# sarulab-speech/visual-onoma-to-wave

Hardware: AMD Instinct MI355X
Metric: end-to-end audio samples/sec (22.05 kHz) + mel-frames/sec, batch 32, 1->8 GPU (higher is better)
Workload: dtype bf16 (encoder+variance adaptor fp32); 1 GPU; C2+C3 end-to-end: vTTS (B, T_src=12, teacher-forced T_mel=512, predicted energy) -> HiFi-GAN V1 generator -> B x 131072 samples; model=vTTS (35.3M) + HiFi-GAN V1 (13.9M), global_batch=32, per_gpu_batch=32, seq_len=512, src_len=12, parallelism=replicas x1 (no data-path collective), pipeline=acoustic(batch i+1) on its own stream || vocoder(batch i)

## Files before the change

### include/vonoma.h

```cpp
#ifndef VONOMA_H_
#define VONOMA_H_

#include <stdint.h>
#ifndef __cplusplus
#include <stdbool.h>
#endif

#ifdef __cplusplus
extern "C" {
#endif

#define VO_OK 0
#define VO_ERR_INVALID (-1)
#define VO_NOT_HANDLED (-2)

enum vo_dtype { VO_F32 = 0, VO_BF16 = 1, VO_F32X3 = 2  };
enum vo_act { VO_ACT_NONE = 0, VO_ACT_RELU = 1, VO_ACT_LRELU = 2, VO_ACT_TANH = 3 };

const char* vo_last_error(void);
#define VO_ABI_VERSION 3
int vo_version(void);
int vo_num_symbols(void);
const char* vo_symbol_name(int i);
int vo_tune(const char* key, int value);
// ... 4 lines not shown
  int64_t x_bstride;
  int ldx;
  const void* w;
  const float* bias;
  void* y;
  int y_dtype;
  int64_t y_bstride;
  int ldy;
  const void* res1;
  const void* res2;
  int B, T_in, T_out;
  int Ci, Co;
  int K, dil, pad;
  int pre_act;  float pre_slope;
  int post_act; float post_slope;
  float out_scale;
  int compute_dtype;
  int transposed, up_stride, up_pad, up_cout, up_tout;
  int variant;
  int stride;
  int groups;
  void* workspace;
  int64_t workspace_bytes;
  const void* ymask;
  float ymask_slope;
  const int32_t* lens;
  int lens_scale;
} vo_conv1d_desc;
int vo_conv1d(const vo_conv1d_desc* d, void* stream);
int64_t vo_conv1d_workspace_size(const vo_conv1d_desc* d);
#define VO_CONV1D_LAUNCH_FIELDS 13
int vo_conv1d_last_launch(int32_t* rec, int n);
int vo_conv1d_plan(const vo_conv1d_desc* d, int32_t* rec, int n);

enum vo_pack_mode { VO_PACK_CONV = 0, VO_PACK_CONVT = 1, VO_PACK_DGRAD = 2 };
int vo_pack_weight(const float* src, const float* g, const float* row_scale, int mode, int Co,
                   int Ci, int K, int stride, void* dst, int dst_dtype, void* stream);

int vo_layernorm(const void* x, int x_dtype, const void* res, int res_dtype, const float* gamma,
                 const float* beta, const int32_t* lens, int B, int T, int D, float eps, void* y,
                 int y_dtype, void* stream);

int vo_layernorm_dual(const void* x, int x_dtype, const void* res, int res_dtype, const float* gamma,
                      const float* beta, const int32_t* lens, int B, int T, int D, float eps, void* y,
                      void* y16, void* stream);

int64_t vo_layernorm_bwd_workspace_size(int B, int T, int D);
int vo_layernorm_bwd(const void* x, const void* res, int x_dtype, const void* gy, int gy_dtype,
                     const float* gamma, const int32_t* lens, int B, int T, int D, float eps, void* gh,
                     float* dgamma, float* dbeta, void* workspace, void* stream);

int vo_layernorm_bwd_ex(const void* x, int x_dtype, const void* res, int res_dtype, const void* gy, int gy_dtype,
                        const void* gy2, const float* gamma, const int32_t* lens, int B, int T, int D, float eps,
                        void* gh, float* gh32, float* dgamma, float* dbeta, void* workspace, void* stream);

int vo_layernorm_drop(const void* x, int x_dtype, const void* res, int res_dtype, const float* gamma,
                      const float* beta, const int32_t* lens, int B, int T, int D, float eps, void* y, int y_dtype,
                      void* y16, float p, const int64_t* seed, unsigned salt, void* stream);
int vo_layernorm_bwd_drop(const void* x, int x_dtype, const void* res, int res_dtype, const void* gy, int gy_dtype,
                          const void* gy2, const float* gamma, const int32_t* lens, int B, int T, int D, float eps,
                          float p, const int64_t* seed, unsigned salt, void* gh, void* gres, float* dgamma,
                          float* dbeta, void* workspace, void* stream);

int vo_attention(const void* qkv, int dtype, const int32_t* lens, int B, int L, int H, int dk,
                 float scale, void* out, void* stream);

// ... 237 lines not shown
```

### visual_onoma_to_wave_amd/_lib.py

```python

import ctypes
import os

_HERE = os.path.dirname(os.path.abspath(__file__))
LIB_PATH = os.environ.get("VO_LIB_PATH") or os.path.join(_HERE, "lib", "libvonoma.so")

VO_F32, VO_BF16, VO_F32X3 = 0, 1, 2
ACT_NONE, ACT_RELU, ACT_LRELU, ACT_TANH = 0, 1, 2, 3
PACK_CONV, PACK_CONVT = 0, 1
HEAD_DURATION, HEAD_ENERGY = 0, 1

c_void_p = ctypes.c_void_p
c_int = ctypes.c_int
c_float = ctypes.c_float
c_int64 = ctypes.c_int64


class Conv1dDesc(ctypes.Structure):
    _fields_ = [
        ("x", c_void_p), ("x_dtype", c_int), ("x_bstride", c_int64), ("ldx", c_int),
        ("w", c_void_p), ("bias", c_void_p),
        ("y", c_void_p), ("y_dtype", c_int), ("y_bstride", c_int64), ("ldy", c_int),
        ("res1", c_void_p), ("res2", c_void_p),
        ("B", c_int), ("T_in", c_int), ("T_out", c_int),
# ... 63 lines not shown
    "vo_num_symbols": (c_int, []),
    "vo_symbol_name": (ctypes.c_char_p, [c_int]),
    "vo_tune": (c_int, [ctypes.c_char_p, c_int]),
    "vo_resblock_pair": (c_int, [c_void_p, c_void_p, c_void_p, c_void_p, c_void_p, c_void_p, c_void_p, c_int,
                                 c_int, c_int, c_int, c_int, c_float, c_float, c_void_p]),
    "vo_resblock_pair_frag": (c_int, [c_void_p, c_void_p, c_void_p, c_void_p, c_void_p, c_void_p, c_void_p, c_int,
                                      c_int, c_int, c_int, c_int, c_float, c_float, c_void_p]),
    "vo_pack_frag": (c_int, [c_void_p, c_void_p, c_int, c_int, c_void_p]),
    "vo_resblock_pair_lens": (c_int, [c_void_p, c_void_p, c_void_p, c_void_p, c_void_p, c_void_p, c_void_p, c_int,
                                      c_int, c_int, c_int, c_int, c_float, c_float, c_void_p, c_void_p, c_int]),
    "vo_resblock_pair_frag_lens": (c_int, [c_void_p, c_void_p, c_void_p, c_void_p, c_void_p, c_void_p, c_void_p, c_int,
                                           c_int, c_int, c_int, c_int, c_float, c_float, c_void_p, c_void_p, c_int]),
    "vo_resblock3_lens": (c_int, [c_void_p, c_void_p, c_void_p, c_void_p, c_void_p, c_void_p, c_void_p, c_void_p, c_int,
                                  c_int, c_int, c_float, c_float, c_void_p, c_void_p, c_int]),
    "vo_conv_post_lens": (c_int, [c_void_p, c_int, c_void_p, c_float, c_int, c_int, c_int, c_int, c_float,
                                  c_void_p, c_void_p, c_void_p, c_int]),
    "vo_conv_post_pcm16": (c_int, [c_void_p, c_int, c_void_p, c_float, c_int, c_int, c_int, c_int, c_float, c_float,
                                   c_void_p, c_void_p]),
    "vo_conv_post_pcm16_lens": (c_int, [c_void_p, c_int, c_void_p, c_float, c_int, c_int, c_int, c_int, c_float,
                                        c_float, c_void_p, c_void_p, c_void_p, c_int]),
    "vo_resblock3": (c_int, [c_void_p, c_void_p, c_void_p, c_void_p, c_void_p, c_void_p, c_void_p, c_void_p, c_int,
                             c_int, c_int, c_float, c_float, c_void_p]),
    "vo_resblockk": (c_int, [c_void_p, c_void_p, c_void_p, c_void_p, c_void_p, c_int, c_void_p, c_void_p, c_void_p,
                             c_int, c_int, c_int, c_float, c_float, c_void_p]),
    "vo_resblockk_lens": (c_int, [c_void_p, c_void_p, c_void_p, c_void_p, c_void_p, c_int, c_void_p, c_void_p, c_void_p,
                                  c_int, c_int, c_int, c_float, c_float, c_void_p, c_void_p, c_int]),
    "vo_resblockk_tile_rows": (c_int, [c_int]),
    "vo_resblock_pair_tile_rows": (c_int, [c_int, c_int, c_int, c_int]),
    "vo_resblock3_tile_rows": (c_int, [c_int, c_void_p]),
    "vo_conv1d": (c_int, [ctypes.POINTER(Conv1dDesc), c_void_p]),
    "vo_conv1d_workspace_size": (ctypes.c_int64, [ctypes.POINTER(Conv1dDesc)]),
    "vo_conv1d_last_launch": (c_int, [ctypes.POINTER(ctypes.c_int32), c_int]),
    "vo_conv1d_plan": (c_int, [ctypes.POINTER(Conv1dDesc), ctypes.POINTER(ctypes.c_int32), c_int]),
    "vo_pack_weight": (c_int, [c_void_p, c_void_p, c_void_p, c_int, c_int, c_int, c_int, c_int,
                               c_void_p, c_int, c_void_p]),
    "vo_layernorm": (c_int, [c_void_p, c_int, c_void_p, c_int, c_void_p, c_void_p, c_void_p, c_int,
                             c_int, c_int, c_float, c_void_p, c_int, c_void_p]),
    "vo_layernorm_dual": (c_int, [c_void_p, c_int, c_void_p, c_int, c_void_p, c_void_p, c_void_p, c_int,
                                  c_int, c_int, c_float, c_void_p, c_void_p, c_void_p]),
    "vo_layernorm_bwd_workspace_size": (ctypes.c_int64, [c_int, c_int, c_int]),
    "vo_layernorm_bwd": (c_int, [c_void_p, c_void_p, c_int, c_void_p, c_int, c_void_p, c_void_p, c_int, c_int,
                                 c_int, c_float, c_void_p, c_void_p, c_void_p, c_void_p, c_void_p]),
    "vo_layernorm_bwd_ex": (c_int, [c_void_p, c_int, c_void_p, c_int, c_void_p, c_int, c_void_p, c_void_p,
                                    c_void_p, c_int, c_int, c_int, c_float, c_void_p, c_void_p, c_void_p,
                                    c_void_p, c_void_p, c_void_p]),
    "vo_layernorm_drop": (c_int, [c_void_p, c_int, c_void_p, c_int, c_void_p, c_void_p, c_void_p, c_int, c_int,
                                  c_int, c_float, c_void_p, c_int, c_void_p, c_float, c_void_p, ctypes.c_uint,
                                  c_void_p]),
    "vo_layernorm_bwd_drop": (c_int, [c_void_p, c_int, c_void_p, c_int, c_void_p, c_int, c_void_p, c_void_p,
                                      c_void_p, c_int, c_int, c_int, c_float, c_float, c_void_p, ctypes.c_uint,
                                      c_void_p, c_void_p, c_void_p, c_void_p, c_void_p, c_void_p]),
    "vo_attention": (c_int, [c_void_p, c_int, c_void_p, c_int, c_int, c_int, c_int, c_float,
                             c_void_p, c_void_p]),
    "vo_attention_bwd_workspace_size": (ctypes.c_int64, [c_int, c_int, c_int]),
    "vo_attention_bwd": (c_int, [c_void_p, c_void_p, c_void_p, c_int, c_void_p, c_int, c_int, c_int, c_int, c_float,
                                 c_void_p, c_void_p, c_void_p]),
    "vo_attention_lse": (c_int, [c_void_p, c_int, c_void_p, c_int, c_int, c_int, c_int, c_float, c_void_p, c_void_p,
                                 c_void_p]),
    "vo_attention_bwd_lse": (c_int, [c_void_p, c_void_p, c_void_p, c_int, c_void_p, c_int, c_int, c_int, c_int,
                                     c_float, c_void_p, c_void_p, c_void_p, c_void_p]),
    "vo_length_regulate": (c_int, [c_void_p, c_int, c_void_p, c_int, c_int, c_int, c_int, c_void_p,
                                   c_int, c_void_p, c_void_p, c_void_p]),
    "vo_length_regulate_bwd": (c_int, [c_void_p, c_int, c_void_p, c_int, c_int, c_int, c_int, c_void_p, c_int,
                                       c_void_p]),
    "vo_lr_lengths": (c_int, [c_void_p, c_int, c_int, c_void_p, c_void_p, c_void_p]),
    "vo_variance_head": (c_int, [ctypes.POINTER(HeadDesc), c_void_p]),
# ... 124 lines not shown
```

### visual_onoma_to_wave_amd/csrc/conv1d.hip

```cpp

#include <string.h>

#include <algorithm>
#include <type_traits>

#include "vo_common.h"

namespace vo {

constexpr int KC = 32;
constexpr int HALO_MAX = 64;

struct ConvArgs {
  const void* x; int64_t xbs; int ldx;
  const void* w; const float* bias;
  void* y; int64_t ybs; int ldy;
  const void* res1; const void* res2;
  int T_in, T_out, Ci, Co, K, dil, pad;
  int pre_act; float pre_slope; int post_act; float post_slope; float out_scale;
  int transposed, up_stride, up_pad, up_cout, up_tout;
  int tiles_per_b, co_tiles, B;
  int cig, cog;
  float* partial;
  int kcs;
// ... 88 lines not shown
      const int pos = min(t0 + wave_t0 + 16 * (j0 + jj) + lr, a.T_out - 1);
      const int64_t off = (int64_t)pos * a.ldy + n0;
#pragma unroll
      for (int h = 0; h < NH; ++h) {
        if (r1) rv1[jj][h] = *reinterpret_cast<const uint4*>(R1 + off + 8 * h);
        if (r2) rv2[jj][h] = *reinterpret_cast<const uint4*>(R2 + off + 8 * h);
        if (om) rvm[jj][h] = *reinterpret_cast<const uint4*>(YM + off + 8 * h);
      }
    }
#pragma unroll
    for (int jj = 0; jj < JG; ++jj) {
      const int j = j0 + jj;
      const int pos = t0 + wave_t0 + 16 * j + lr;
      const int64_t off = (int64_t)min(pos, a.T_out - 1) * a.ldy + n0;
#pragma unroll
      for (int h = 0; h < NH; ++h) {
        float q[8], x1[8], x2[8];
        if (r1) {
          const uint32_t w[4] = {rv1[jj][h].x, rv1[jj][h].y, rv1[jj][h].z, rv1[jj][h].w};
#pragma unroll
          for (int u = 0; u < 4; ++u) {
            x1[2 * u] = __uint_as_float(w[u] << 16);
            x1[2 * u + 1] = __uint_as_float(w[u] & 0xffff0000u);
          }
        }
        if (r2) {
          const uint32_t w[4] = {rv2[jj][h].x, rv2[jj][h].y, rv2[jj][h].z, rv2[jj][h].w};
#pragma unroll
          for (int u = 0; u < 4; ++u) {
            x2[2 * u] = __uint_as_float(w[u] << 16);
            x2[2 * u + 1] = __uint_as_float(w[u] & 0xffff0000u);
          }
        }
#pragma unroll
        for (int e = 0; e < 8; ++e) {
          const int i = 2 * h + e / 4, r = e & 3;
          float v = acc[i][j][r] + bias[8 * h + e];
          v = tanh_act ? tanhf(v) : lrelu_max(v, ps);
          if (r1) v += x1[e];
          v *= a.out_scale;
          if (r2) v += x2[e];
          q[e] = v;
        }
        if (om) {
          const uint32_t w[4] = {rvm[jj][h].x, rvm[jj][h].y, rvm[jj][h].z, rvm[jj][h].w};
#pragma unroll
          for (int e = 0; e < 8; ++e) {
            const float m = __uint_as_float((e & 1) ? (w[e >> 1] & 0xffff0000u) : (w[e >> 1] << 16));
            const float r = to_f32(from_f32<bf16_t>(q[e]));
            q[e] = m > 0.f ? r : r * a.ymask_slope;
          }
        }
        if (pos < a.T_out) store8(Y + off + 8 * h, q);
      }
    }
  }
}

template <typename TOUT, int NI, int NJ, int EJ = 2>
__device__ __forceinline__ void conv_epilogue(const ConvArgs& a, f32x4 (&acc)[NI][NJ], int b, int t0, int co_blk,
                                              int wave_co0, int wave_t0, int lane) {
  const int lr = lane & 15;
  const int g = lane >> 4;
  const int n0 = co_blk + wave_co0 + NI * 4 * g;
  if (n0 >= a.Co) return;
  if constexpr (std::is_same<TOUT, bf16_t>::value && NI % 2 == 0) {
    if (!a.transposed && (a.ldy & 7) == 0 && (a.ybs & 7) == 0 && a.Co % (4 * NI) == 0) {
      conv_epilogue_vec<NI, NJ, EJ>(a, acc, b, t0, n0, wave_t0, lr);
      return;
    }
  }
  TOUT* Y = reinterpret_cast<TOUT*>(a.y) + (int64_t)b * a.ybs;
  const TOUT* R1 = a.res1 ? reinterpret_cast<const TOUT*>(a.res1) + (int64_t)b * a.ybs : nullptr;
  const TOUT* R2 = a.res2 ? reinterpret_cast<const TOUT*>(a.res2) + (int64_t)b * a.ybs : nullptr;

  int col = n0, trow_shift = 0;
// ... 668 lines not shown
  bool SEG = false;
  constexpr int bco() const { return 16 * NI * WCO; }
  constexpr int bt() const { return 16 * NJ * WT; }
  constexpr Tile role(int r, int prio = 0) const { Tile t = *this; t.ROLE = r; t.PRIO = prio; return t; }
  constexpr Tile dma(bool rs = false) const { Tile t = *this; t.GL = true; t.RS = rs; return t; }
  constexpr Tile tps(int n) const { Tile t = *this; t.TPS = n; return t; }
  constexpr Tile seg() const { Tile t = *this; t.SEG = true; return t; }
};
constexpr Tile T32x16{1, 1, 2, 1, 4}, T64x16{1, 1, 4, 1, 4}, T128x16{2, 1, 4, 1, 4}, T128x32{2, 2, 4, 1, 4},
    T128x32_n4w2{4, 1, 2, 2, 2}, T32x64{2, 1, 1, 4, 4}, T64x64{2, 2, 2, 2, 2}, T64x64_n4w1{4, 1, 1, 4, 4},
    T128x64{4, 2, 2, 2, 2}, T64x128{2, 4, 2, 2, 2}, T64x128_n4w1{4, 2, 1, 4, 4}, T128x128{4, 4, 2, 2, 2},
    T256x128{4, 4, 4, 2, 2}, T32x256{2, 4, 1, 4, 4}, T64x256{4, 4, 1, 4, 4}, T128x256{4, 4, 2, 4, 2}, T256x256{4, 8, 4, 2, 2};
constexpr Tile T32x64_seg = Tile{1, 2, 2, 2, 1}.seg(), T64x64_seg = Tile{2, 2, 2, 2, 1}.seg(),
               T32x128_seg = Tile{1, 4, 2, 2, 1}.seg(), T64x128_seg = Tile{2, 4, 2, 2, 1}.seg();
constexpr Tile T256x256_mrf0 = T256x256.role(1, 1).dma(), T256x256_mrf0_rs = T256x256.role(1, 1).dma(true),
               T128x128_mrf1 = T128x128.role(2), T64x256_mrf2 = T64x256.role(3), T32x256_mrf3 = T32x256.role(4);
#ifdef VO_ABLATIONS
constexpr Tile A256x256_t1_gl = T256x256.tps(1).dma(), A256x256_t1_rs = T256x256.tps(1).dma(true),
               A128x128_t1_gl = T128x128.tps(1).dma(), A256x256_t1 = T256x256.tps(1), A64x128_t1 = T64x128.tps(1),
               A128x128_mrf0 = T128x128.role(1), A256x256_mrf0_plain = T256x256.role(1),
               A256x256_mrf0_prio = T256x256.role(1, 1), A256x256_mrf0_t3 = T256x256.role(1, 1).tps(3).dma(),
               A256x256_mrf0_t1 = T256x256.role(1, 1).tps(1).dma(), A256x256_mrf0_t1_rs = T256x256.role(1, 1).tps(1).dma(true);
constexpr Tile LIN_64x64{2, 2, 2, 2, 0}, LIN_128x128{4, 4, 2, 2, 0}, LIN_64x128{2, 4, 2, 2, 0}, LIN_128x64{4, 2, 2, 2, 0};
#define VO_AB(...) , __VA_ARGS__
#else
#define VO_AB(...)
#endif

enum ConvTypes { FFF, FXF, BBB, BBF, FBB, FBF };
constexpr int kTypeBytes[][3] = {{4, 4, 4}, {4, 4, 4}, {2, 2, 2}, {2, 2, 4}, {4, 2, 2}, {4, 2, 4}};

struct ConvPlan {
  bool ups;
  int types, role;
  const Tile* tile;
  int S;
  bool nice;
  int splits, kcs;
  size_t lds;
};

static ConvArgs conv_args(const vo_conv1d_desc* d, int BCO, int BT) {
  ConvArgs a;
  memset(&a, 0, sizeof(a));
  a.x = d->x; a.xbs = d->x_bstride; a.ldx = d->ldx; a.w = d->w; a.bias = d->bias;
  a.y = d->y; a.ybs = d->y_bstride; a.ldy = d->ldy; a.res1 = d->res1; a.res2 = d->res2;
  a.T_in = d->T_in; a.T_out = d->T_out; a.Ci = d->Ci; a.Co = d->Co; a.K = d->K; a.dil = d->dil; a.pad = d->pad;
  a.pre_act = d->pre_act; a.pre_slope = d->pre_slope;
  a.post_act = d->post_act; a.post_slope = d->post_slope; a.out_scale = d->out_scale;
  a.transposed = d->transposed; a.up_stride = d->up_stride; a.up_pad = d->up_pad; a.up_cout = d->up_cout; a.up_tout = d->up_tout;
  a.tiles_per_b = (d->T_out + BT - 1) / BT;
  a.co_tiles = (d->Co + BCO - 1) / BCO;
  a.B = d->B;
  a.ymask = d->ymask; a.ymask_slope = d->ymask_slope;
  a.lens = d->lens; a.lens_scale = d->lens_scale;
  const int groups = d->groups > 1 ? d->groups : 1;
  a.cig = d->Ci / groups;
  a.cog = d->Co / groups;
  return a;
}

template <const Tile& T, typename TIN, typename TC, typename TOUT, bool RAG = false, int S = 1>
static int launch_tile(const vo_conv1d_desc* d, const ConvPlan& p, hipStream_t st) {
  constexpr int BT = T.bt(), TPS = sizeof(TC) == 2 ? T.TPS : 1;
  ConvArgs a = conv_args(d, T.bco(), BT);
  if (T.SEG) a.tiles_per_b = 1;
// ... 168 lines not shown
static int launch_types(const vo_conv1d_desc* d, const ConvPlan& p, hipStream_t st) {
  int rc = kNoTile;
  if constexpr (sizeof(TC) == 4) rc = launch_among<TIN, TC, TOUT, false, 1, T32x64_seg, T64x64_seg, T32x128_seg, T64x128_seg>(d, p, st);
  if constexpr (sizeof(TC) == 2)
    rc = launch_among<TIN, TC, TOUT, RAG, 1, T64x128, T256x128, T128x256, T256x256 VO_AB(
        A256x256_t1_gl, A256x256_t1_rs, A128x128_t1_gl, A256x256_t1, A64x128_t1)>(d, p, st);
#ifdef VO_ABLATIONS
  if constexpr (sizeof(TC) == 2 && sizeof(TIN) == 2)
    if (p.tile->TPS == 0)
      return d->Ci == 256 ? launch_lin_tile<TOUT, 8>(d, p.tile, st)
                          : d->Ci == 512 ? launch_lin_tile<TOUT, 16>(d, p.tile, st) : launch_lin_tile<TOUT, 32>(d, p.tile, st);
#endif
  if (rc != kNoTile) return rc;
  return launch_among<TIN, TC, TOUT, RAG, 1, T32x16, T64x16, T128x16, T128x32, T32x256, T64x256, T64x128_n4w1, T64x64_n4w1,
                      T64x64, T128x128>(d, p, st);
}

template <typename TIN, typename TC, typename TOUT, int S>
static int launch_disc_s(const vo_conv1d_desc* d, const ConvPlan& p, hipStream_t st) {
  if constexpr (S >= 8) return launch_among<TIN, TC, TOUT, false, S, T128x32_n4w2, T32x64, T64x64_n4w1, T128x64>(d, p, st);
  return launch_among<TIN, TC, TOUT, false, S, T32x64, T64x64_n4w1, T128x64>(d, p, st);
}
template <typename TIN, typename TC, typename TOUT>
static int launch_disc(const vo_conv1d_desc* d, const ConvPlan& p, hipStream_t st) {
  switch (p.S) {
    case 1: return launch_disc_s<TIN, TC, TOUT, 1>(d, p, st);
    case 2: return launch_disc_s<TIN, TC, TOUT, 2>(d, p, st);
    case 3: return launch_disc_s<TIN, TC, TOUT, 3>(d, p, st);
    case 4: return launch_disc_s<TIN, TC, TOUT, 4>(d, p, st);
    default: return launch_disc_s<TIN, TC, TOUT, 8>(d, p, st);
  }
}

static int launch_plan(const vo_conv1d_desc* d, const ConvPlan& p, hipStream_t st) {
  const bool rag = d->lens != nullptr;
  int rc = kNoTile;
  if (d->stride > 1 || d->groups > 1)
    rc = p.types == FFF ? launch_disc<float, float, float>(d, p, st)
                        : p.types == BBB ? launch_disc<bf16_t, bf16_t, bf16_t>(d, p, st) : launch_disc<bf16_t, bf16_t, float>(d, p, st);
  else if (p.role && rag)
    rc = launch_among<bf16_t, bf16_t, bf16_t, true, 1, T256x256_mrf0, T256x256_mrf0_rs>(d, p, st);
  else if (p.role)
    rc = launch_among<bf16_t, bf16_t, bf16_t, false, 1, T256x256_mrf0, T256x256_mrf0_rs, T128x128_mrf1, T64x256_mrf2, T32x256_mrf3 VO_AB(
        A128x128_mrf0, A256x256_mrf0_plain, A256x256_mrf0_prio, A256x256_mrf0_t3, A256x256_mrf0_t1, A256x256_mrf0_t1_rs)>(d, p, st);
  else switch (p.types) {
    case FXF: rc = launch_types<float, bx3_t, float>(d, p, st); break;
    case FFF: rc = rag ? launch_types<float, float, float, true>(d, p, st) : launch_types<float, float, float>(d, p, st); break;
    case BBB: rc = rag ? launch_types<bf16_t, bf16_t, bf16_t, true>(d, p, st) : launch_types<bf16_t, bf16_t, bf16_t>(d, p, st); break;
    case FBB: rc = rag ? launch_types<float, bf16_t, bf16_t, true>(d, p, st) : launch_types<float, bf16_t, bf16_t>(d, p, st); break;
    case BBF: rc = launch_types<bf16_t, bf16_t, float>(d, p, st); break;
    default: rc = launch_types<float, bf16_t, float>(d, p, st);
  }
  if (rc == kNoTile) vo_set_error("conv1d: the selected tile is not compiled for type triple %d", p.types);
  return rc == kNoTile ? VO_ERR_INVALID : rc;
}

bool vo_ups_takes(const vo_conv1d_desc* d);
int vo_ups_launch(const vo_conv1d_desc* d, hipStream_t st);

static int conv1d_check(const vo_conv1d_desc* d, ConvPlan* p) {
  VO_CHECK_ARG(d != nullptr, "conv1d: null descriptor");
  VO_CHECK_ARG(d->x && d->w && d->y, "conv1d: null tensor pointer");
  VO_CHECK_ARG((d->pre_act != VO_ACT_LRELU || (d->pre_slope >= 0.f && d->pre_slope <= 1.f)) &&
                   (d->post_act != VO_ACT_LRELU || (d->post_slope >= 0.f && d->post_slope <= 1.f)),
               "conv1d: leaky-ReLU slope outside [0, 1]");
  VO_CHECK_ARG(d->B > 0 && d->T_in > 0 && d->T_out > 0 && d->Ci > 0 && d->Co > 0 && d->K > 0,
               "conv1d: non-positive size (B=%d T_in=%d T_out=%d Ci=%d Co=%d K=%d)", d->B, d->T_in, d->T_out, d->Ci, d->Co, d->K);
// ... 39 lines not shown
    p->types = FXF;
    return VO_OK;
  }
  if (d->stride > 1 || d->groups > 1) {
    const int g = d->groups > 1 ? d->groups : 1;
    VO_CHECK_ARG(!d->transposed && d->variant == 0, "conv1d: stride/groups exclude transposed and variants");
    VO_CHECK_ARG(d->Ci % g == 0 && d->Co % g == 0, "conv1d: Ci %d / Co %d not divisible by groups %d", d->Ci, d->Co, g);
    if (d->compute_dtype != VO_F32) {
      VO_CHECK_ARG(d->compute_dtype == VO_BF16 && xi == VO_BF16, "conv1d: strided/grouped bf16 needs bf16 input");
      p->types = yo == VO_BF16 ? BBB : BBF;
      return VO_OK;
    }
  }
  if (d->compute_dtype == VO_F32) {
    VO_CHECK_ARG(xi == VO_F32 && yo == VO_F32, "conv1d: fp32 compute needs fp32 I/O");
    p->types = FFF;
    return VO_OK;
  }
  VO_CHECK_ARG(d->compute_dtype == VO_BF16, "conv1d: bad compute dtype");
  if (d->lens) {
    VO_CHECK_ARG(yo == VO_BF16 && d->variant <= 1, "conv1d: lens with bf16 compute needs a bf16 output, variant 0 / 1");
    p->types = xi == VO_F32 ? FBB : BBB;
  } else if ((xi != VO_BF16 && xi != VO_F32) || (yo != VO_BF16 && yo != VO_F32)) {
    vo_set_error("conv1d: bad dtypes");
    return VO_ERR_INVALID;
  } else {
    p->types = xi == VO_BF16 ? (yo == VO_BF16 ? BBB : BBF) : (yo == VO_BF16 ? FBB : FBF);
  }
  p->role = p->types == BBB ? d->variant : 0;
  return VO_OK;
}

static int conv1d_plan(const vo_conv1d_desc* d, ConvPlan* p) {
  const int rc = conv1d_check(d, p);
  if (rc != VO_OK || p->ups) return rc;
  p->S = d->stride > 1 ? d->stride : 1;
  p->tile = d->stride > 1 || d->groups > 1 ? select_disc(d) : p->role ? select_role(d, p->role)
                                           : select_types(d, kTypeBytes[p->types][0], kTypeBytes[p->types][1]);
  return p->tile ? plan_tile(d, p) : VO_ERR_INVALID;
}

}

using namespace vo;

extern "C" int64_t vo_conv1d_workspace_size(const vo_conv1d_desc* d) {
  int splits = 1, kcs = 0;
  if (!d || !splitk_plan(d, &splits, &kcs)) return 0;
  return (int64_t)splits * d->B * d->T_out * d->Co * (int64_t)sizeof(float);
}

static int copy_record(const int32_t* src, int32_t* rec, int n) {
  const int m = rec ? std::max(0, std::min(n, (int)VO_CONV1D_LAUNCH_FIELDS)) : 0;
  if (m > 0) memcpy(rec, src, m * sizeof(int32_t));
  return m;
}

extern "C" int vo_conv1d_last_launch(int32_t* rec, int n) { return copy_record(g_last_launch, rec, n); }

extern "C" int vo_conv1d_plan(const vo_conv1d_desc* d, int32_t* rec, int n) {
  int32_t r[VO_CONV1D_LAUNCH_FIELDS] = {};
  ConvPlan p;
  const int rc = conv1d_plan(d, &p);
  if (rc == VO_OK) plan_record(d, p, r);
  copy_record(r, rec, n);
  return rc;
}

// ... 11 lines not shown
```

### visual_onoma_to_wave_amd/csrc/vo_common.h

```cpp
#pragma once

#include <hip/hip_runtime.h>
#include <hip/hip_bf16.h>
#include <stdint.h>

#include "../../include/vonoma.h"

typedef unsigned short bf16_t;
typedef __bf16 bf16x8 __attribute__((ext_vector_type(8)));
typedef float f32x4 __attribute__((ext_vector_type(4)));

namespace vo {

__device__ __forceinline__ float to_f32(float x) { return x; }
__device__ __forceinline__ float to_f32(bf16_t x) { return __uint_as_float(((uint32_t)x) << 16); }

template <typename T> __device__ __forceinline__ T from_f32(float x);
template <> __device__ __forceinline__ float from_f32<float>(float x) { return x; }
template <> __device__ __forceinline__ bf16_t from_f32<bf16_t>(float x) {
  __hip_bfloat16 b = __float2bfloat16(x);
  return *reinterpret_cast<bf16_t*>(&b);
}

typedef __bf16 bf16x2_t __attribute__((ext_vector_type(2)));
typedef float f32x2_t __attribute__((ext_vector_type(2)));
__device__ __forceinline__ uint32_t pk_bf16(float lo, float hi) {
  return __builtin_bit_cast(uint32_t, __builtin_convertvector((f32x2_t){lo, hi}, bf16x2_t));
}
__device__ __forceinline__ float lrelu_max(float v, float s) { return __builtin_elementwise_maximum(v, v * s); }

__device__ __forceinline__ int table_find(const int* start, int n, int x) {
  int lo = 0, hi = n - 1;
  while (lo < hi) {
    const int mid = (lo + hi + 1) >> 1;
    if (start[mid] <= x) lo = mid; else hi = mid - 1;
  }
  return lo;
}

__device__ __forceinline__ int rag_rows(const int32_t* lens, int scale, int b, int T) {
  const int64_t r = (int64_t)max(lens[b], 0) * scale;
  return (int)min(r, (int64_t)T);
}

__device__ __forceinline__ int xcd_grouped_id(int w, int n) {
  const int x = w & 7, k = w >> 3, q = n >> 3, r = n & 7;
  return x * q + (x < r ? x : r) + k;
}

__device__ __forceinline__ void lds_barrier() { asm volatile("s_waitcnt lgkmcnt(0)\n\ts_barrier" ::: "memory"); }

__device__ __forceinline__ uint32_t drop_mix(uint32_t h) {
  h ^= h >> 16; h *= 0x85ebca6bu; h ^= h >> 13; h *= 0xc2b2ae35u; h ^= h >> 16;
  return h;
}
__device__ __forceinline__ uint32_t drop_hash(uint32_t s0, uint32_t s1, uint32_t i) {
  return drop_mix(drop_mix(i * 0x9E3779B9u ^ s0) + s1);
}
__device__ __forceinline__ void drop_keys(const int64_t* seed, uint32_t salt, uint32_t& s0, uint32_t& s1) {
  const uint64_t sd = (uint64_t)seed[0];
  s0 = (uint32_t)sd ^ drop_mix(salt + 0x3C6EF372u);
  s1 = (uint32_t)(sd >> 32);
// ... 162 lines not shown
```

### visual_onoma_to_wave_amd/csrc/vo_runtime.cpp

```cpp
#include <stdarg.h>
#include <stdio.h>
#include <stdlib.h>
#include <string.h>

#include "../../include/vonoma.h"

static thread_local char g_err[512] = "";

extern "C" void vo_set_error(const char* fmt, ...) {
  va_list ap;
  va_start(ap, fmt);
  vsnprintf(g_err, sizeof(g_err), fmt, ap);
  va_end(ap);
}

extern "C" const char* vo_last_error(void) { return g_err; }

extern "C" int vo_version(void) { return VO_ABI_VERSION; }

static const char* const kKnobs[] = {"pair_cfg", "conv_cfg", "gen_cfg", "wgrad_cfg", "rb3_cfg", "att_cfg", "ups_cfg", "post_cfg", "splitk_cfg",
                                      "wgrad_mt", "wgrad_kg", "att_xcd", "pc_cfg", "rs_cfg", "lin_cfg", "seg_cfg", "tile_cfg"};
static int g_knobs[sizeof(kKnobs) / sizeof(kKnobs[0])] = {};

static bool is_ablation(const char* key, int value);
// ... 37 lines not shown
      return VO_OK;
    }
  vo_set_error("vo_tune: unknown key %s", key ? key : "(null)");
  return VO_ERR_INVALID;
}

extern "C" int vo_tune_get(const char* key) {
  knobs_from_env();
  for (size_t i = 0; i < sizeof(kKnobs) / sizeof(kKnobs[0]); ++i)
    if (!strcmp(key, kKnobs[i])) return g_knobs[i];
  return 0;
}

static const char* const kSymbols[] = {
    "vo_last_error",     "vo_version",       "vo_num_symbols", "vo_symbol_name",   "vo_conv1d",
    "vo_pack_weight",    "vo_layernorm",     "vo_layernorm_dual",     "vo_attention",   "vo_length_regulate", "vo_lr_lengths",
    "vo_variance_head",  "vo_vfe_stencil",   "vo_add_pos_class", "vo_conv_post",   "vo_transpose_bct",
    "vo_stft_mel",       "vo_mask_from_lengths", "vo_tune", "vo_resblock_pair", "vo_stft_mel_ex",
    "vo_pack_grouped",   "vo_pack_grouped_blocks", "vo_period_fold",   "vo_wav_cl8",     "vo_avgpool_wav",  "vo_gan_reduce",
    "vo_gan_reduce_grad", "vo_glyph_batch", "vo_char_features",
    "vo_conv1d_wgrad",   "vo_colsum",        "vo_conv1d_wgrad_grouped", "vo_resblock3",
    "vo_layernorm_bwd_workspace_size", "vo_layernorm_bwd", "vo_layernorm_bwd_ex", "vo_layernorm_drop", "vo_layernorm_bwd_drop", "vo_attention_bwd_workspace_size", "vo_attention_bwd",
    "vo_length_regulate_bwd", "vo_conv1d_wgrad_bias", "vo_lrelu_mask", "vo_conv1d_workspace_size",
    "vo_bn_workspace_size", "vo_bn_train_fwd", "vo_bn_bwd", "vo_vfe_conv_workspace_size", "vo_vfe_conv_fwd",
    "vo_vfe_conv_bwd", "vo_stft_mel_bwd_workspace_size", "vo_stft_mel_bwd", "vo_period_fold_bwd", "vo_wav_cl8_bwd",
    "vo_avgpool_wav_bwd", "vo_weight_norm", "vo_weight_norm_bwd", "vo_pack_dgrad_phase", "vo_pack_batch", "vo_seq_remap", "vo_seq_remap2", "vo_lrelu_mask_add", "vo_lrelu_mask_sum", "vo_spectral_norm", "vo_gan_reduce_multi", "vo_gan_reduce_multi_workspace_size", "vo_gan_reduce_grad_multi", "vo_spectral_norm_bwd", "vo_spectral_norm_bwd_workspace_size", "vo_conv1d_wgrad_workspace_size", "vo_colsum_workspace_size", "vo_stft_mag",
    "vo_stft_mag_bwd_workspace_size", "vo_stft_mag_bwd", "vo_stft_loss", "vo_stft_loss_grad",
    "vo_bucket_embed",   "vo_embed_bwd",     "vo_adam_multi",  "vo_opt_step_increment",
    "vo_resblock_pair_frag", "vo_pack_frag", "vo_attention_lse", "vo_attention_bwd_lse", "vo_dropout",
    "vo_conv1d_last_launch", "vo_conv1d_plan", "vo_conv1d_wgrad_last_launch", "vo_conv1d_wgrad_plan",
    "vo_resblock_pair_lens", "vo_resblock_pair_frag_lens", "vo_resblock3_lens", "vo_conv_post_lens",
    "vo_resblockk", "vo_resblockk_lens", "vo_resblockk_tile_rows", "vo_resblock_pair_tile_rows", "vo_resblock3_tile_rows",
    "vo_vfe_stencil_lds_bytes", "vo_vfe_stencil_ex", "vo_vfe_conv_workspace_size_ex", "vo_vfe_conv_fwd_ex", "vo_vfe_conv_bwd_ex",
    "vo_variance_head_ctl", "vo_conv_post_pcm16", "vo_conv_post_pcm16_lens",
};

extern "C" int vo_num_symbols(void) { return (int)(sizeof(kSymbols) / sizeof(kSymbols[0])); }
extern "C" const char* vo_symbol_name(int i) {
  return (i >= 0 && i < vo_num_symbols()) ? kSymbols[i] : nullptr;
}
```

### visual_onoma_to_wave_amd/ops.py

```python

import ctypes

import numpy as np

import torch

from . import _lib, profiling
from ._lib import (ACT_LRELU, ACT_NONE, ACT_RELU, ACT_TANH, HEAD_DURATION, HEAD_ENERGY,
                   PACK_CONV, PACK_CONVT, VO_BF16, VO_F32, VO_F32X3)

_DT = {torch.float32: VO_F32, torch.bfloat16: VO_BF16}


class _F32X3:

    def __repr__(self):
        return "ops.F32X3"


F32X3 = _F32X3()


def storage_dtype(cdt):
    return torch.float32 if cdt is F32X3 else cdt
# ... 116 lines not shown

def conv1d(x, w_packed, bias, *, tag=None, **kw):
    d, x, out, ws_bytes = _conv1d_desc(x, w_packed, bias, **kw)
    if ws_bytes > 0:
        ws = torch.empty(ws_bytes // 4, dtype=torch.float32, device=x.device)
        d.workspace, d.workspace_bytes = ws.data_ptr(), ws_bytes
    timer = profiling.active()
    ev = timer.start() if (tag is not None and timer is not None and timer.watching(tag)) else None
    _lib.check(_lib.lib().vo_conv1d(ctypes.byref(d), _stream(x)), "vo_conv1d")
    if ev is not None:
        res1, res2 = kw.get("res1"), kw.get("res2")
        flops = 2.0 * d.B * d.T_out * d.Co * d.Ci * d.K / kw.get("groups", 1)
        nbytes = (d.B * d.T_in * d.Ci * x.element_size() + out.numel() * out.element_size() +
                  (res1.numel() * res1.element_size() if res1 is not None else 0) +
                  (res2.numel() * res2.element_size() if res2 is not None else 0) +
                  w_packed.numel() * w_packed.element_size())
        timer.stop(tag, ev, flops, nbytes, kernel=f"conv1d_kernel<..., ROLE={d.variant}>")
    return out


LAUNCH_FIELDS = ("BCO", "BT", "S", "SEG", "nice", "splits", "sizeof_in", "sizeof_compute", "sizeof_out", "ROLE",
                 "compute_dtype", "NI", "WCO")


def conv1d_plan(x, w_packed, bias, *, tag=None, **kw):
    d, x, _, ws_bytes = _conv1d_desc(x, w_packed, bias, **kw)
    if ws_bytes > 0:
        d.workspace, d.workspace_bytes = d.y, ws_bytes
    rec = (ctypes.c_int32 * len(LAUNCH_FIELDS))()
    _lib.check(_lib.lib().vo_conv1d_plan(ctypes.byref(d), rec, len(LAUNCH_FIELDS)), "vo_conv1d_plan")
    return dict(zip(LAUNCH_FIELDS, (int(v) for v in rec)))


def conv1d_last_launch():
    rec = (ctypes.c_int32 * len(LAUNCH_FIELDS))()
    n = _lib.lib().vo_conv1d_last_launch(rec, len(LAUNCH_FIELDS))
    if n != len(LAUNCH_FIELDS):
        raise RuntimeError(f"vo_conv1d_last_launch returned {n} fields, expected {len(LAUNCH_FIELDS)}")
    return dict(zip(LAUNCH_FIELDS, (int(v) for v in rec)))


def pack_dgrad_weight(w, dtype):
    w = w.detach().float().contiguous()
    Co, Ci, K = w.shape
    out = torch.empty((K, Ci, Co), dtype=dtype, device=w.device)
    _lib.check(_lib.lib().vo_pack_weight(_ptr(w), None, None, 2, Co, Ci, K, 1, _ptr(out), vo_dtype(dtype),
                                         _stream(w)), "vo_pack_weight")
    return out


def pack_conv_weight(w, dtype, g=None, row_scale=None, transposed_stride=None):
    w = w.detach().float().contiguous()
    if transposed_stride is None:
        Co, Ci, K = w.shape
        out = torch.empty((K, Co, Ci), dtype=dtype, device=w.device)
        mode, stride = PACK_CONV, 1
    else:
        Ci, Co, K = w.shape
        s = transposed_stride
        out = torch.empty((2, s * Co, Ci), dtype=dtype, device=w.device)
        mode, stride = PACK_CONVT, s
    g = None if g is None else g.detach().float().reshape(-1).contiguous()
    rs = None if row_scale is None else row_scale.detach().float().reshape(-1).contiguous()
    _lib.check(_lib.lib().vo_pack_weight(_ptr(w), _ptr(g), _ptr(rs), mode, Co, Ci, K, stride,
                                         _ptr(out), vo_dtype(dtype), _stream(w)), "vo_pack_weight")
    return out
# ... 1232 lines not shown
```

Before: 365.2 million audio samples/s.

## Add software-pipelined plane conv kernel for 256-channel MRF bf16 convs

Measured after the change: 379.9 million audio samples/s, median of 6. 1.04x the previous value.

```diff
diff --git a/include/vonoma.h b/include/vonoma.h
--- a/include/vonoma.h
+++ b/include/vonoma.h
@@ -60,6 +60,7 @@
 #define VO_CONV1D_LAUNCH_FIELDS 13
 int vo_conv1d_last_launch(int32_t* rec, int n);
 int vo_conv1d_plan(const vo_conv1d_desc* d, int32_t* rec, int n);
+int vo_conv1d_plane_takes(const vo_conv1d_desc* d);
 
 enum vo_pack_mode { VO_PACK_CONV = 0, VO_PACK_CONVT = 1, VO_PACK_DGRAD = 2 };
 int vo_pack_weight(const float* src, const float* g, const float* row_scale, int mode, int Co,
diff --git a/visual_onoma_to_wave_amd/_lib.py b/visual_onoma_to_wave_amd/_lib.py
--- a/visual_onoma_to_wave_amd/_lib.py
+++ b/visual_onoma_to_wave_amd/_lib.py
@@ -119,6 +119,7 @@
     "vo_conv1d_workspace_size": (ctypes.c_int64, [ctypes.POINTER(Conv1dDesc)]),
     "vo_conv1d_last_launch": (c_int, [ctypes.POINTER(ctypes.c_int32), c_int]),
     "vo_conv1d_plan": (c_int, [ctypes.POINTER(Conv1dDesc), ctypes.POINTER(ctypes.c_int32), c_int]),
+    "vo_conv1d_plane_takes": (c_int, [ctypes.POINTER(Conv1dDesc)]),
     "vo_pack_weight": (c_int, [c_void_p, c_void_p, c_void_p, c_int, c_int, c_int, c_int, c_int,
                                c_void_p, c_int, c_void_p]),
     "vo_layernorm": (c_int, [c_void_p, c_int, c_void_p, c_int, c_void_p, c_void_p, c_void_p, c_int,
diff --git a/visual_onoma_to_wave_amd/csrc/conv1d.hip b/visual_onoma_to_wave_amd/csrc/conv1d.hip
--- a/visual_onoma_to_wave_amd/csrc/conv1d.hip
+++ b/visual_onoma_to_wave_amd/csrc/conv1d.hip
@@ -144,16 +144,13 @@
             x2[2 * u + 1] = __uint_as_float(w[u] & 0xffff0000u);
           }
         }
+        float av[8], bv[8];
 #pragma unroll
         for (int e = 0; e < 8; ++e) {
-          const int i = 2 * h + e / 4, r = e & 3;
-          float v = acc[i][j][r] + bias[8 * h + e];
-          v = tanh_act ? tanhf(v) : lrelu_max(v, ps);
-          if (r1) v += x1[e];
-          v *= a.out_scale;
-          if (r2) v += x2[e];
-          q[e] = v;
+          av[e] = acc[2 * h + e / 4][j][e & 3];
+          bv[e] = bias[8 * h + e];
         }
+        conv_epilogue8(av, bv, tanh_act, ps, r1, x1, a.out_scale, r2, x2, q);
         if (om) {
           const uint32_t w[4] = {rvm[jj][h].x, rvm[jj][h].y, rvm[jj][h].z, rvm[jj][h].w};
 #pragma unroll
@@ -888,6 +885,7 @@
 
 struct ConvPlan {
   bool ups;
+  bool plane;
   int types, role;
   const Tile* tile;
   int S;
@@ -1122,7 +1120,10 @@
   }
 }
 
+int vo_conv_plane_launch(const vo_conv1d_desc* d, hipStream_t st);
+
 static int launch_plan(const vo_conv1d_desc* d, const ConvPlan& p, hipStream_t st) {
+  if (p.plane) return vo_conv_plane_launch(d, st);
   const bool rag = d->lens != nullptr;
   int rc = kNoTile;
   if (d->stride > 1 || d->groups > 1)
@@ -1228,8 +1229,10 @@
 }
 
 static int conv1d_plan(const vo_conv1d_desc* d, ConvPlan* p) {
+  p->plane = false;
   const int rc = conv1d_check(d, p);
   if (rc != VO_OK || p->ups) return rc;
+  p->plane = p->role == 1 && vo_conv1d_plane_takes(d) != 0;
   p->S = d->stride > 1 ? d->stride : 1;
   p->tile = d->stride > 1 || d->groups > 1 ? select_disc(d) : p->role ? select_role(d, p->role)
                                            : select_types(d, kTypeBytes[p->types][0], kTypeBytes[p->types][1]);
diff --git a/visual_onoma_to_wave_amd/csrc/conv_plane.hip b/visual_onoma_to_wave_amd/csrc/conv_plane.hip
--- /dev/null
+++ b/visual_onoma_to_wave_amd/csrc/conv_plane.hip
@@ -0,0 +1,248 @@
+
+#include "mrf_plane.h"
+
+namespace vo {
+
+struct CplArgs {
+  const bf16_t* x; const bf16_t* w; const float* bias; bf16_t* y; const bf16_t* res1; const bf16_t* res2;
+  int64_t xbs, ybs;
+  int T, dil, pad, tiles_per_b;
+  float pre_slope, ps, out_scale;
+  unsigned long long* stamps;
+};
+
+constexpr int CPL_C = 256, CPL_R = 256;
+constexpr int CPL_WR = CPL_R + 64;
+constexpr int CPL_PL = CPL_WR * 32;
+constexpr int CPL_NPB = 4;
+constexpr size_t CPL_LDS = (size_t)CPL_NPB * CPL_PL * sizeof(bf16_t) + CPL_C * sizeof(float);
+constexpr int CPL_NSTW = 16, CPL_NPT = 16;
+
+template <int K, bool ST = false>
+__global__ void __launch_bounds__(256, 1) mrf_conv_plane_kernel(CplArgs a) {
+  constexpr int C = CPL_C, NC = C / 32, NJ = 16, NS = CPL_WR / 64;
+  constexpr int PL = CPL_PL, NPB = CPL_NPB;
+  constexpr int NA = 6, DA = NA - 1;
+  constexpr int TG = K < DA ? K : DA;
+  constexpr int NPC = NC * K, P0 = NPC - TG;
+  constexpr int NQ = NPC * NJ;
+  constexpr int NB = 6, DB = 4;
+  constexpr int NR = 4, RD = 3;
+  static_assert(K >= 3 && TG >= 3 && NA > DA && NR > RD && DB <= NJ, "conv plane: schedule");
+
+  const int T = a.T, dil = a.dil;
+
+  extern __shared__ __attribute__((aligned(16))) char smem_raw[];
+  bf16_t* win = reinterpret_cast<bf16_t*>(smem_raw);
+  float* sbias = reinterpret_cast<float*>(win + NPB * PL);
+
+  const int tid = threadIdx.x, lane = tid & 63;
+  const int w = __builtin_amdgcn_readfirstlane(tid >> 6);
+  const int lr = lane & 15, lg = lane >> 4;
+  const int b = blockIdx.x / a.tiles_per_b;
+  const int t0 = (blockIdx.x - b * a.tiles_per_b) * CPL_R;
+  auto stamp = [&](int idx) {
+    if constexpr (ST) {
+      if (blockIdx.x < CPL_NSTW && lane == 0)
+        a.stamps[(blockIdx.x * 4 + w) * CPL_NPT + idx] = __builtin_amdgcn_s_memtime();
+    }
+  };
+  stamp(0);
+
+  sbias[tid] = a.bias[tid];
+
+  const int aoff = ((64 * w + 16 * (lr >> 2) + (lr & 3)) * C + 8 * lg) * (int)sizeof(bf16_t);
+  const __amdgpu_buffer_rsrc_t rw = __builtin_amdgcn_make_buffer_rsrc((void*)a.w, (short)0, K * C * C * 2, 0x00020000);
+  bf16x8 A[NA][4];
+  auto loadA = [&](int p, int i) {
+    const int c = p / K, k = p % K;
+    A[p % NA][i] = __builtin_bit_cast(bf16x8, __builtin_amdgcn_raw_buffer_load_b128(rw, aoff + i * 4 * C * 2 + c * 64,
+                                                                                     k * (C * C * 2), 0));
+  };
+
+  const int srow = tid >> 2, sq = tid & 3;
+  const int xl = plane_off(srow, sq);
+  const __amdgpu_buffer_rsrc_t rsx = plane_utt<C>(a.x + b * a.xbs, 0, T, T);
+  const int wneed = CPL_R + (K - 1) * dil;
+  int xo[NS];
+#pragma unroll
+  for (int s = 0; s < NS; ++s)
+    xo[s] = srow + 64 * s < wneed ? ((t0 - a.pad + srow + 64 * s) * C + 8 * sq) * 2 : 0x7ffffff0;
+  u32x4 xw[2][NS];
+  const float pre_slope = a.pre_slope;
+  auto load_win = [&](int c, int s) { xw[c & 1][s] = __builtin_amdgcn_raw_buffer_load_b128(rsx, xo[s] + c * 64, 0, 0); };
+  auto store_win = [&](int c, int s) {
+    *reinterpret_cast<u32x4*>(win + (c % NPB) * PL + xl + s * 64 * 32) = lrelu8(xw[c & 1][s], pre_slope);
+  };
+
+  const int valid = min(CPL_R, T - t0);
+  const int64_t ybase = b * a.ybs + (int64_t)t0 * C;
+  const bool r1 = a.res1 != nullptr, r2 = a.res2 != nullptr;
+  const __amdgpu_buffer_rsrc_t yrs =
+      __builtin_amdgcn_make_buffer_rsrc((void*)(a.y + ybase), (short)0, valid * C * 2, 0x00020000);
+  const __amdgpu_buffer_rsrc_t r1s =
+      __builtin_amdgcn_make_buffer_rsrc((void*)((r1 ? a.res1 : a.y) + ybase), (short)0, r1 ? valid * C * 2 : 0, 0x00020000);
+  const __amdgpu_buffer_rsrc_t r2s =
+      __builtin_amdgcn_make_buffer_rsrc((void*)((r2 ? a.res2 : a.y) + ybase), (short)0, r2 ? valid * C * 2 : 0, 0x00020000);
+  const int eoff = (lr * C + 64 * w + 16 * lg) * 2;
+  u32x4 rv1[NR][2], rv2[NR][2];
+  auto load_res = [&](int j) {
+#pragma unroll
+    for (int h = 0; h < 2; ++h) {
+      rv1[j % NR][h] = __builtin_amdgcn_raw_buffer_load_b128(r1s, eoff + j * 16 * C * 2 + 16 * h, 0, 0);
+      rv2[j % NR][h] = __builtin_amdgcn_raw_buffer_load_b128(r2s, eoff + j * 16 * C * 2 + 16 * h, 0, 0);
+    }
+  };
+
+#pragma unroll
+  for (int p = 0; p < DA; ++p)
+#pragma unroll
+    for (int i = 0; i < 4; ++i) loadA(p, i);
+#pragma unroll
+  for (int s = 0; s < NS; ++s) load_win(0, s);
+#pragma unroll
+  for (int s = 0; s < NS; ++s) load_win(1, s);
+#pragma unroll
+  for (int s = 0; s < NS; ++s) store_win(0, s);
+#pragma unroll
+  for (int s = 0; s < NS; ++s) load_win(2, s);
+
+  f32x4 acc[4][NJ];
+  bf16x8 Bq[NB];
+  int tb[K];
+#pragma unroll
+  for (int k = 0; k < K; ++k) tb[k] = plane_off(k * dil + lr, lg);
+
+  auto chunk_of = [&](int q) { return q < P0 * NJ ? q / NJ / K : NC - 1; };
+  auto tap_of = [&](int q) { return q < P0 * NJ ? (q / NJ) % K : K - TG + (q - P0 * NJ) % TG; };
+  auto rt_of = [&](int q) { return q < P0 * NJ ? q % NJ : (q - P0 * NJ) / TG; };
+  auto readB = [&](int q) {
+    Bq[q % NB] = *reinterpret_cast<const bf16x8*>(win + (chunk_of(q) % NPB) * PL + tb[tap_of(q)] + rt_of(q) * 512);
+  };
+
+  const float ps = a.ps, osc = a.out_scale;
+  auto post = [&](int j, int h) {
+    float av[8], bv[8], x1[8], x2[8], q[8];
+    const f32x4 b0 = *reinterpret_cast<const f32x4*>(sbias + 64 * w + 16 * lg + 8 * h);
+    const f32x4 b1 = *reinterpret_cast<const f32x4*>(sbias + 64 * w + 16 * lg + 8 * h + 4);
+#pragma unroll
+    for (int e = 0; e < 8; ++e) {
+      av[e] = acc[2 * h + e / 4][j][e & 3];
+      bv[e] = e < 4 ? b0[e & 3] : b1[e & 3];
+    }
+    unpack8(rv1[j % NR][h], x1);
+    unpack8(rv2[j % NR][h], x2);
+    conv_epilogue8(av, bv, false, ps, r1, x1, osc, r2, x2, q);
+    const u32x4 v = u32x4{pk_bf16(q[0], q[1]), pk_bf16(q[2], q[3]), pk_bf16(q[4], q[5]), pk_bf16(q[6], q[7])};
+    __builtin_amdgcn_raw_buffer_store_b128(v, yrs, eoff + j * 16 * C * 2 + 16 * h, 0, 0);
+  };
+
+  lds_barrier();
+  stamp(1);
+#pragma unroll
+  for (int q = 0; q < DB; ++q) readB(q);
+
+#pragma unroll
+  for (int q = 0; q < NQ; ++q) {
+    const int c = chunk_of(q), k = tap_of(q), j = rt_of(q);
+    const bool tail = q >= P0 * NJ;
+    const int p = tail ? NPC : q / NJ;
+    if (q % (K * NJ) == 0) stamp(2 + c);
+    if (q == P0 * NJ) stamp(2 + NC);
+    if (q + DB < NQ) readB(q + DB);
+    if (!tail) {
+      if (j < 4 && p + DA < NPC) loadA(p + DA, j);
+      if (k == 0 && c + 1 < NC && j >= 5 && j % 2 == 1 && (j - 5) / 2 < NS) store_win(c + 1, (j - 5) / 2);
+      if (k == 1 && c + 3 < NC && j >= 4 && j % 2 == 0 && (j - 4) / 2 < NS) load_win(c + 3, (j - 4) / 2);
+      if (p == P0 - 1 && j >= 10 && j - 10 < RD) load_res(j - 10);
+    }
+    __builtin_amdgcn_sched_barrier(0);
+    const bf16x8 bq = Bq[q % NB];
+    const bf16x8(&Ak)[4] = A[(c * K + k) % NA];
+    if (c == 0 && k == 0) {
+#pragma unroll
+      for (int i = 0; i < 4; ++i)
+        acc[i][j] = __builtin_amdgcn_mfma_f32_16x16x32_bf16(Ak[i], bq, f32x4{0.f, 0.f, 0.f, 0.f}, 0, 0, 0);
+    } else {
+#pragma unroll
+      for (int i = 0; i < 4; ++i) acc[i][j] = __builtin_amdgcn_mfma_f32_16x16x32_bf16(Ak[i], bq, acc[i][j], 0, 0, 0);
+    }
+    if (tail) {
+      const int kk = (q - P0 * NJ) % TG;
+      if (j > 0 && kk == 1) post(j - 1, 0);
+      if (j > 0 && kk == 2) post(j - 1, 1);
+      if (kk == 2 && j + RD < NJ) load_res(j + RD);
+    }
+    __builtin_amdgcn_sched_barrier(0);
+    if (!tail && k == 0 && j == NJ - 1 && c + 1 < NC) lds_barrier();
+  }
+  stamp(3 + NC);
+  post(NJ - 1, 0);
+  post(NJ - 1, 1);
+  stamp(4 + NC);
+}
+
+template <int K>
+static int cpl_launch(const CplArgs& a, int B, hipStream_t st) {
+  hipLaunchKernelGGL(mrf_conv_plane_kernel<K>, dim3((unsigned)(a.tiles_per_b * B)), dim3(256), CPL_LDS, st, a);
+  VO_RETURN_LAUNCH();
+}
+
+static CplArgs cpl_args(const vo_conv1d_desc* d) {
+  CplArgs a;
+  a.x = (const bf16_t*)d->x; a.w = (const bf16_t*)d->w; a.bias = d->bias; a.y = (bf16_t*)d->y;
+  a.res1 = (const bf16_t*)d->res1; a.res2 = (const bf16_t*)d->res2;
+  a.xbs = d->x_bstride; a.ybs = d->y_bstride;
+  a.T = d->T_out; a.dil = d->dil; a.pad = d->pad;
+  a.tiles_per_b = (d->T_out + CPL_R - 1) / CPL_R;
+  a.pre_slope = d->pre_act == VO_ACT_LRELU ? d->pre_slope : 1.f;
+  a.ps = d->post_act == VO_ACT_LRELU ? d->post_slope : 1.f;
+  a.out_scale = d->out_scale;
+  a.stamps = nullptr;
+  return a;
+}
+
+int vo_conv_plane_launch(const vo_conv1d_desc* d, hipStream_t st) {
+  const CplArgs a = cpl_args(d);
+  return d->K == 3 ? cpl_launch<3>(a, d->B, st) : d->K == 7 ? cpl_launch<7>(a, d->B, st) : cpl_launch<11>(a, d->B, st);
+}
+
+}
+
+using namespace vo;
+
+extern "C" int vo_conv1d_plane_takes(const vo_conv1d_desc* d) {
+  if (!d || !d->x || !d->w || !d->y || !d->bias) return 0;
+  if (d->variant != 1 || d->x_dtype != VO_BF16 || d->y_dtype != VO_BF16 || d->compute_dtype != VO_BF16) return 0;
+  if (d->Ci != CPL_C || d->Co != CPL_C || d->ldx != CPL_C || d->ldy != CPL_C) return 0;
+  if (!(d->K == 3 || d->K == 7 || d->K == 11) || d->dil < 1 || (d->K - 1) * d->dil > 64) return 0;
+  if (2 * d->pad != (d->K - 1) * d->dil || d->T_out != d->T_in || d->T_in < 1 || d->B < 1) return 0;
+  if (d->stride > 1 || d->groups > 1 || d->transposed || d->ymask || d->workspace || d->lens) return 0;
+  if (!(d->pre_act == VO_ACT_NONE || d->pre_act == VO_ACT_LRELU)) return 0;
+  if (!(d->post_act == VO_ACT_NONE || d->post_act == VO_ACT_LRELU)) return 0;
+  if (vo_tune_get("conv_cfg") != 0) return 0;
+  if (d->x_bstride % 8 != 0 || d->y_bstride % 8 != 0) return 0;
+  if (((int64_t)d->T_in + CPL_WR) * CPL_C * 2 >= ((int64_t)1 << 31)) return 0;
+  if ((int64_t)d->B * ((d->T_out + CPL_R - 1) / CPL_R) >= ((int64_t)1 << 31)) return 0;
+  return 1;
+}
+
+#ifdef VO_CPL_STAMPS
+extern "C" int vo_cpl_stamps(const vo_conv1d_desc* d, unsigned long long* host_out) {
+  if (!vo_conv1d_plane_takes(d)) return -1;
+  const size_t n = (size_t)CPL_NSTW * 4 * CPL_NPT;
+  unsigned long long* dev = nullptr;
+  if (hipMalloc(&dev, n * 8) != hipSuccess) return -1;
+  (void)hipMemset(dev, 0, n * 8);
+  CplArgs a = cpl_args(d);
+  a.stamps = dev;
+  const dim3 grid((unsigned)(a.tiles_per_b * d->B));
+  if (d->K == 3) hipLaunchKernelGGL((mrf_conv_plane_kernel<3, true>), grid, dim3(256), CPL_LDS, 0, a);
+  else if (d->K == 7) hipLaunchKernelGGL((mrf_conv_plane_kernel<7, true>), grid, dim3(256), CPL_LDS, 0, a);
+  else hipLaunchKernelGGL((mrf_conv_plane_kernel<11, true>), grid, dim3(256), CPL_LDS, 0, a);
+  (void)hipDeviceSynchronize();
+  (void)hipMemcpy(host_out, dev, n * 8, hipMemcpyDeviceToHost);
+  (void)hipFree(dev);
+  return 0;
+}
+#endif
diff --git a/visual_onoma_to_wave_amd/csrc/vo_common.h b/visual_onoma_to_wave_amd/csrc/vo_common.h
--- a/visual_onoma_to_wave_amd/csrc/vo_common.h
+++ b/visual_onoma_to_wave_amd/csrc/vo_common.h
@@ -28,6 +28,20 @@
   return __builtin_bit_cast(uint32_t, __builtin_convertvector((f32x2_t){lo, hi}, bf16x2_t));
 }
 __device__ __forceinline__ float lrelu_max(float v, float s) { return __builtin_elementwise_maximum(v, v * s); }
+
+__device__ __forceinline__ void conv_epilogue8(const float (&acc)[8], const float (&bias)[8], bool tanh_act, float ps,
+                                               bool r1, const float (&x1)[8], float scale, bool r2,
+                                               const float (&x2)[8], float (&q)[8]) {
+#pragma unroll
+  for (int e = 0; e < 8; ++e) {
+    float v = acc[e] + bias[e];
+    v = tanh_act ? tanhf(v) : lrelu_max(v, ps);
+    if (r1) v += x1[e];
+    v *= scale;
+    if (r2) v += x2[e];
+    q[e] = v;
+  }
+}
 
 __device__ __forceinline__ int table_find(const int* start, int n, int x) {
   int lo = 0, hi = n - 1;
diff --git a/visual_onoma_to_wave_amd/csrc/vo_runtime.cpp b/visual_onoma_to_wave_amd/csrc/vo_runtime.cpp
--- a/visual_onoma_to_wave_amd/csrc/vo_runtime.cpp
+++ b/visual_onoma_to_wave_amd/csrc/vo_runtime.cpp
@@ -93,7 +93,7 @@
     "vo_resblock_pair_lens", "vo_resblock_pair_frag_lens", "vo_resblock3_lens", "vo_conv_post_lens",
     "vo_resblockk", "vo_resblockk_lens", "vo_resblockk_tile_rows", "vo_resblock_pair_tile_rows", "vo_resblock3_tile_rows",
     "vo_vfe_stencil_lds_bytes", "vo_vfe_stencil_ex", "vo_vfe_conv_workspace_size_ex", "vo_vfe_conv_fwd_ex", "vo_vfe_conv_bwd_ex",
-    "vo_variance_head_ctl", "vo_conv_post_pcm16", "vo_conv_post_pcm16_lens",
+    "vo_variance_head_ctl", "vo_conv_post_pcm16", "vo_conv_post_pcm16_lens", "vo_conv1d_plane_takes",
 };
 
 extern "C" int vo_num_symbols(void) { return (int)(sizeof(kSymbols) / sizeof(kSymbols[0])); }
diff --git a/visual_onoma_to_wave_amd/ops.py b/visual_onoma_to_wave_amd/ops.py
--- a/visual_onoma_to_wave_amd/ops.py
+++ b/visual_onoma_to_wave_amd/ops.py
@@ -172,6 +172,13 @@
     return dict(zip(LAUNCH_FIELDS, (int(v) for v in rec)))
 
 
+def conv1d_plane_takes(x, w_packed, bias, *, tag=None, **kw):
+    d, x, _, ws_bytes = _conv1d_desc(x, w_packed, bias, **kw)
+    if ws_bytes > 0:
+        d.workspace, d.workspace_bytes = d.y, ws_bytes
+    return bool(_lib.lib().vo_conv1d_plane_takes(ctypes.byref(d)))
+
+
 def conv1d_last_launch():
     rec = (ctypes.c_int32 * len(LAUNCH_FIELDS))()
     n = _lib.lib().vo_conv1d_last_launch(rec, len(LAUNCH_FIELDS))
```
